# teamtomo/torch-motion-correction

Hardware: AMD Instinct MI355X
Metric: frames/sec motion-corrected, 40×4k×4k fp32 stack, 1/2/4/8 MI355X (higher is better)
Workload: dtype f32; 1 GPU; 40-frame 4096x4096 fp32 movie, global rigid shift estimate+correct (estimate_global_motion -> correct_motion, frames + sum out), 1 stack per GPU per step, consecutive steps overlapped on two HIP streams; b_factor=500

## Files before the change

### torch_motion_correction_amd/csrc/mc_wave_fft.h

```cpp
#pragma once

#ifdef __HIPCC__
#include "mc_common.h"
#define MC_HD __host__ __device__ __forceinline__
#else
#include <math.h>
#include <stdint.h>
struct cfloat {
  float x, y;
};
#define MC_HD static inline
#endif

typedef float wf2 __attribute__((ext_vector_type(2)));

#define WF_N 2048
#define WF_SLAB 1024

#ifdef __HIPCC__
__device__ __forceinline__ void wf_sync() {
  __builtin_amdgcn_fence(__ATOMIC_RELEASE, "wavefront");
  __builtin_amdgcn_wave_barrier();
  __builtin_amdgcn_fence(__ATOMIC_ACQUIRE, "wavefront");
}
// ... 49 lines not shown
  a2 = t0 - t2;
  a1 = wf_add_mi(t1, d);
  a3 = wf_sub_mi(t1, d);
}

MC_HD void wf_dft16(wf2 (&a)[16]) {
  const float C1 = 0.92387953251128673848f, S1 = 0.38268343236508978178f;
  const float H = 0.70710678118654752440f;
#pragma unroll
  for (int j = 0; j < 4; ++j) wf_bfly4(a[j], a[j + 4], a[j + 8], a[j + 12]);
  a[1 + 4] = wf_cmulc(a[1 + 4], C1, -S1);
  a[1 + 8] = wf_cmulc(a[1 + 8], H, -H);
  a[1 + 12] = wf_cmulc(a[1 + 12], S1, -C1);
  a[2 + 4] = wf_cmulc(a[2 + 4], H, -H);
  a[2 + 12] = wf_cmulc(a[2 + 12], -H, -H);
  a[3 + 4] = wf_cmulc(a[3 + 4], S1, -C1);
  a[3 + 8] = wf_cmulc(a[3 + 8], -H, -H);
  a[3 + 12] = wf_cmulc(a[3 + 12], -C1, S1);
#pragma unroll
  for (int p = 0; p < 4; ++p) {
    wf2 &b0 = a[4 * p], &b1 = a[4 * p + 1], &b2 = a[4 * p + 2], &b3 = a[4 * p + 3];
    if (p == 2) {
      const wf2 t0 = wf_add_mi(b0, b2), t1 = wf_sub_mi(b0, b2);
      const wf2 t2 = b1 + b3, d = b1 - b3;
      b0 = t0 + t2;
      b2 = t0 - t2;
      b1 = wf_add_mi(t1, d);
      b3 = wf_sub_mi(t1, d);
    } else {
      wf_bfly4(b0, b1, b2, b3);
    }
  }
#pragma unroll
  for (int p = 0; p < 4; ++p)
#pragma unroll
    for (int r = p + 1; r < 4; ++r) {
      const wf2 s = a[4 * p + r];
      a[4 * p + r] = a[4 * r + p];
      a[4 * r + p] = s;
    }
}

MC_HD void wf_dft16_lo2(wf2 (&a)[16]) {
  const float C1 = 0.92387953251128673848f, S1 = 0.38268343236508978178f;
  const float H = 0.70710678118654752440f;
  const wf2 x0 = a[0], x1 = a[1], x2 = a[14], x3 = a[15];
  a[0] = x0; a[4] = x0; a[8] = x0; a[12] = x0;
  a[1] = x1;
  a[1 + 4] = wf_cmulc(x1, C1, -S1);
  a[1 + 8] = wf_cmulc(x1, H, -H);
  a[1 + 12] = wf_cmulc(x1, S1, -C1);
  a[2] = x2;
  a[2 + 4] = wf_cmulc(x2, H, H);
  a[2 + 8] = -x2;
  a[2 + 12] = wf_cmulc(x2, -H, H);
  a[3] = x3;
  a[3 + 4] = wf_cmulc(x3, C1, S1);
  a[3 + 8] = wf_cmulc(x3, H, H);
  a[3 + 12] = wf_cmulc(x3, S1, C1);
#pragma unroll
  for (int p = 0; p < 4; ++p) {
    wf2 &b0 = a[4 * p], &b1 = a[4 * p + 1], &b2 = a[4 * p + 2], &b3 = a[4 * p + 3];
    if (p == 2) {
      const wf2 t0 = wf_add_mi(b0, b2), t1 = wf_sub_mi(b0, b2);
      const wf2 t2 = b1 + b3, d = b1 - b3;
      b0 = t0 + t2;
      b2 = t0 - t2;
      b1 = wf_add_mi(t1, d);
      b3 = wf_sub_mi(t1, d);
    } else {
      wf_bfly4(b0, b1, b2, b3);
    }
  }
#pragma unroll
  for (int p = 0; p < 4; ++p)
#pragma unroll
    for (int r = p + 1; r < 4; ++r) {
      const wf2 s = a[4 * p + r];
      a[4 * p + r] = a[4 * r + p];
      a[4 * r + p] = s;
    }
}

template <int KEEP>
MC_HD void wf_dft8_pruned(const wf2 (&e)[4], const wf2 (&o)[4], wf2 (&z)[8]) {
  const float H = 0.70710678118654752440f;
  wf2 e0 = e[0], e1 = e[1], e2 = e[2], e3 = e[3];
  wf2 o0 = o[0], o1 = o[1], o2 = o[2], o3 = o[3];
  wf_bfly4(e0, e1, e2, e3);
  wf_bfly4(o0, o1, o2, o3);
  z[0] = e0 + o0;
  z[7] = wf_fma_c(e3, o3, H, H);
  if (KEEP >= 2) {
    z[1] = wf_fma_c(e1, o1, H, -H);
    z[6] = wf_sub_mi(e2, o2);
  }
  if (KEEP >= 4) {
    z[2] = wf_add_mi(e2, o2);
    z[3] = wf_fma_c(e3, o3, -H, -H);
    z[4] = e0 - o0;
    z[5] = wf_fma_c(e1, o1, -H, H);
  }
}

struct WfLane {
  int x1w_base, x1w_mask;
  int x1r[4];
  int x2w;
  int x2r[4];
  int kbin[4];
  int self;
};

MC_HD WfLane wf_lane(int t) {
  WfLane L;
  {
    const int n2 = t >> 2, h1 = (t >> 1) & 1, h0 = t & 1;
    L.x1w_base = (n2 * 2 + h1) * 32 + h0 * 16;
    L.x1w_mask = (n2 & 3) | (h1 << 2) | (h0 << 3);
  }
  {
    const int k1 = t & 15, g2 = t >> 4, h1 = g2 >> 1, h0 = g2 & 1;
    const int lanepart = h1 * 32 + h0 * 16, lo = k1 ^ ((h1 << 2) | (h0 << 3));
    for (int v = 0; v < 4; ++v) L.x1r[v] = lanepart + (lo ^ v);
    L.x2w = g2 * 256 + k1;
  }
  L.kbin[0] = t;
  L.kbin[1] = t == 0 ? 128 : 256 - t;
  L.kbin[2] = 64 + t;
  L.kbin[3] = 192 - t;
  for (int s = 0; s < 4; ++s) L.x2r[s] = L.kbin[s];
  L.self = t == 0;
  return L;
}

MC_HD wf2 wf_unpack(wf2 zk, wf2 zmr, wf2 wk) {
  const wf2 zm = {zmr.x, -zmr.y};
  const wf2 sm = zk + zm, d = zk - zm;
  const wf2 wd = wf_cmul(d, wk);
  return wf_add_mi(sm, wd) * 0.5f;
}

template <int KEEP>
MC_HD void wf_unpack_lane(const wf2 (&z)[4][8], const wf2 (&wk)[4], bool self, wf2 (&X)[4][KEEP]) {
  const float C1 = 0.92387953251128673848f, S1 = 0.38268343236508978178f;
#pragma unroll
  for (int k3 = 0; k3 < KEEP; ++k3) {
    const wf2 m_a0 = self ? z[0][(8 - k3) & 7] : z[1][7 - k3];
    const wf2 m_a1 = self ? z[1][7 - k3] : z[0][7 - k3];
    wf2 w[4] = {wk[0], wk[1], wk[2], wk[3]};
    if (k3 == 1) {
#pragma unroll
      for (int s = 0; s < 4; ++s) w[s] = wf_cmulc(w[s], C1, -S1);
    }
    X[0][k3] = wf_unpack(z[0][k3], m_a0, w[0]);
    X[1][k3] = wf_unpack(z[1][k3], m_a1, w[1]);
    X[2][k3] = wf_unpack(z[2][k3], z[3][7 - k3], w[2]);
    X[3][k3] = wf_unpack(z[3][k3], z[2][7 - k3], w[3]);
  }
}

#define WF5_N 512
#define WF5_SLAB 512

MC_HD void wf_dft8(wf2 (&a)[8]) {
  const float H = 0.70710678118654752440f;
// ... 41 lines not shown
```

### torch_motion_correction_amd/csrc/xc_common.h

```cpp
#pragma once
#include <string.h>
#include "mc_fft.h"
#include "mcorr.h"

struct XcGeom {
  int W, H;
  int nkx;
  int kyp, kyn;
  int y0, ny;
  int x0, x1;
  int RG;
};

struct XcBox {
  int hl, hu, wl, wu;
};

__device__ __forceinline__ int kept_index(int ky, int H, int kyp, int kyn) {
  if (ky < kyp) return ky;
  if (ky >= H - kyn) return ky - (H - kyn) + kyp;
  return -1;
}

struct PeakCand {
  float v;
  int idx;
};
__device__ __forceinline__ void cand_merge(float& bv, int& bi, float v, int i) {
  if (v > bv || (v == bv && i < bi)) {
    bv = v;
    bi = i;
  }
}

__device__ __forceinline__ int float_order(float f) {
  const int i = __float_as_int(f);
  return i >= 0 ? i : i ^ 0x7fffffff;
}

#define MC_DISPATCH_CASE(V, ...) \
  case V: {                      \
    constexpr int L = V;         \
    __VA_ARGS__;                 \
  } break;
#define MC_DISPATCH_LOG(LOGV, ...)          \
  switch (LOGV) {                           \
    MC_DISPATCH_CASE(4, __VA_ARGS__)        \
    MC_DISPATCH_CASE(5, __VA_ARGS__)        \
    MC_DISPATCH_CASE(6, __VA_ARGS__)        \
    MC_DISPATCH_CASE(7, __VA_ARGS__)        \
    MC_DISPATCH_CASE(8, __VA_ARGS__)        \
    MC_DISPATCH_CASE(9, __VA_ARGS__)        \
    MC_DISPATCH_CASE(10, __VA_ARGS__)       \
    MC_DISPATCH_CASE(11, __VA_ARGS__)       \
    MC_DISPATCH_CASE(12, __VA_ARGS__)       \
    default:                                \
      return MC_ERR_UNSUPPORTED;            \
  }

static int geom_from(const mc_xc_geom* q, XcGeom* g, bool rows_pow2 = true, bool cols_pow2 = true) {
  if (!q) return MC_ERR_ARG;
  if (q->W < 4 || q->W > 16384 || ((q->W & 1) && q->W > 8191) || q->H < 2 || q->H > 8192) return MC_ERR_UNSUPPORTED;
  if (rows_pow2 && (!mc_is_pow2(q->W) || q->W < 32 || q->W > 8192)) return MC_ERR_UNSUPPORTED;
  if (cols_pow2 && (!mc_is_pow2(q->H) || q->H < 16 || q->H > 4096)) return MC_ERR_UNSUPPORTED;
  if (q->nkx < 1 || q->nkx > q->W / 2 + 1) return MC_ERR_ARG;
  if (q->kyp < 0 || q->kyn < 0 || q->kyp + q->kyn < 1 || q->kyp + q->kyn > q->H) return MC_ERR_ARG;
  if (q->RG < 1 || q->ny < 1 || q->ny % q->RG || q->H % q->RG) return MC_ERR_ARG;
  if (rows_pow2 && (q->RG % (MC_WG / fft_threads(q->W / 2)))) return MC_ERR_ARG;
  if (q->y0 < 0 || q->y0 + q->ny > q->H) return MC_ERR_ARG;
  if (q->x0 < 0 || q->x1 > q->W || q->x0 >= q->x1) return MC_ERR_ARG;
  if (!(q->W & 1) && ((q->x0 & 1) || (q->x1 & 1))) return MC_ERR_ARG;
  g->W = q->W; g->H = q->H; g->nkx = q->nkx; g->kyp = q->kyp; g->kyn = q->kyn;
  g->y0 = q->y0; g->ny = q->ny; g->x0 = q->x0; g->x1 = q->x1; g->RG = q->RG;
  return MC_OK;
}

static inline size_t rows_lds_bytes(int N, const XcGeom& g) {
  const int sgroups = MC_WG / fft_threads(N);
  return sizeof(cfloat) * ((size_t)sgroups * 2 * lds_len(N) + (size_t)g.nkx * (g.RG + 1));
}
template <typename Kernel>
static inline int mc_dyn_lds(Kernel kernel, size_t lds) {
  if (lds > 160 * 1024) return MC_ERR_ARG;
  if (lds > 64 * 1024)
    (void)hipFuncSetAttribute((const void*)kernel, hipFuncAttributeMaxDynamicSharedMemorySize, (int)lds);
  return MC_OK;
}

static inline int xc_near_groups(const XcGeom& g) {
  const int ngrp = g.H / g.RG, near = (64 + g.RG - 1) / g.RG;
  return 2 * near > ngrp ? ngrp / 2 : near;
}

void mc_launch_row_bounds(const cfloat* T2, float* bounds, int nkx, int H, int npairs, hipStream_t stream);
void mc_launch_peak_final(const float* part_val, const int* part_idx, int ngrp, int H, int W, int* peaks,
                          float* shifts, const int* shift_rows, int npairs, hipStream_t stream);

__attribute__((visibility("hidden"))) int mc_launch_cols_inv_near(const cfloat* S_cur, const int* cur_idx, const cfloat* S_ref, const int* ref_idx,
                            cfloat* T2n, float* bounds, const cfloat* tw_col, float scale, const XcGeom& g, int nstore,
                            int npairs, hipStream_t stream);
__attribute__((visibility("hidden"))) int mc_launch_cols_inv_gated(const cfloat* S_cur, const int* cur_idx, const cfloat* S_ref, const int* ref_idx,
                             cfloat* T2, const cfloat* tw_col, float scale, const XcGeom& g, const int* gate,
                             int npairs, hipStream_t stream);
```

### torch_motion_correction_amd/csrc/xc_rows_fwd.hip

```cpp
#include "xc_rows_fwd.h"

template <typename T>
__global__ __launch_bounds__(256) void xc_provisional_mean_kernel(const T* __restrict__ x, int n,
                                                                  float* __restrict__ m0) {
  double s = 0.0;
  for (int i = threadIdx.x; i < n; i += 256) s += (double)(float)x[i];
  for (int off = 32; off > 0; off >>= 1) s += __shfl_down(s, off);
  __shared__ double part[4];
  if ((threadIdx.x & 63) == 0) part[threadIdx.x >> 6] = s;
  __syncthreads();
  if (threadIdx.x == 0) {
    m0[0] = (float)(((part[0] + part[1]) + (part[2] + part[3])) / (double)n);
    m0[1] = 1.f;
    m0[2] = 1.f;
  }
}

__global__ void xc_stats_finalize(const double* __restrict__ acc_slots, double count,
                                  const float* __restrict__ m0, float* __restrict__ fix,
                                  float* __restrict__ out3) {
  double acc[2] = {0.0, 0.0};
  for (int s = 0; s < XC_STAT_SLOTS; ++s) {
    acc[0] += acc_slots[2 * s];
    acc[1] += acc_slots[2 * s + 1];
  }
  const double dm = acc[0] / count;
  double var = (acc[1] - acc[0] * acc[0] / count) / (count - 1.0);
  if (var < 0) var = 0;
  const float stdf = (float)sqrt(var);
  fix[0] = (float)dm;
  fix[1] = 1.0f / stdf;
  out3[0] = (float)((double)m0[0] + dm);
  out3[1] = 1.0f / stdf;
  out3[2] = stdf;
}

__global__ __launch_bounds__(256) void xc_rows_hot_fix(const long long* __restrict__ keys, const float2* __restrict__ rv,
                                                       int64_t n, int frame0, int njobs, int h, int w,
                                                       const float* __restrict__ mask,
                                                       const float* __restrict__ mean_rstd, cfloat* __restrict__ T1,
                                                       int W, int nkx, int y0, int ny) {
#pragma clang fp contract(off)
  const int64_t e0 = blockIdx.x;
  if (e0 >= n) return;
  const long long seg = keys[e0] / w;
  if (e0 > 0 && keys[e0 - 1] / w == seg) return;
  const int f = (int)(seg / h), y = (int)(seg - (long long)f * h);
  if (f < frame0 || f >= frame0 + njobs || y < y0 || y >= y0 + ny) return;
  const float rstd = mean_rstd[1];
  cfloat* col = T1 + (int64_t)(f - frame0) * nkx * ny + (y - y0);
  for (int kx = threadIdx.x; kx < nkx; kx += 256) {
    float ar = 0.f, ai = 0.f;
    for (int64_t e = e0; e < n && keys[e] / w == seg; ++e) {
      const int x = (int)(keys[e] - seg * w);
      const float m = mask ? mask[(int64_t)y * w + x] : 1.f;
      if (m == 0.f) continue;
      const float2 p = rv[e];
      const float dA = (p.x - p.y) * rstd * m;
      const int ph = (int)(((int64_t)kx * x) % W);
      const float rev = (float)ph / (float)W;
      ar += dA * __builtin_amdgcn_cosf(rev);
      ai -= dA * __builtin_amdgcn_sinf(rev);
    }
    cfloat* o = col + (int64_t)kx * ny;
    o->x += ar;
    o->y += ai;
  }
}

static int g_row_engine = 0;

enum K1Engine { K1_WAVE, K1_WG, K1_NONE };
static K1Engine k1_route(const XcGeom& g, int raw, bool half, const void* src, const float* gain, const float* mask,
                         const int* job_expo, int64_t row_stride, const XcBox& b, bool stats) {
  const bool shape = g.W == 2 * WF_N && g.nkx <= 512 && (g.ny % 8) == 0;
  const bool aligned16 = ((reinterpret_cast<uintptr_t>(src) | reinterpret_cast<uintptr_t>(gain) |
                           reinterpret_cast<uintptr_t>(mask)) & 15) == 0;
  if (raw) return shape && aligned16 && (row_stride & 7) == 0 ? K1_WAVE : K1_WG;
  const bool wave = shape && mask && !job_expo && aligned16 && (row_stride & 3) == 0 &&
                    (!stats || ((b.wl | b.wu) & 255) == 0);
  if (half && !wave) return K1_NONE;
  return wave && g_row_engine != 1 ? K1_WAVE : K1_WG;
}

static K1WaveVariant k1_wave_variant(const XcGeom& g, int raw, bool half, const int* row_chord) {
  const bool inner = g.x0 >= 256 && g.x0 <= 512 && g.x1 >= 3584 && g.x1 <= 3840;
  if (half) return K1WaveVariant{g.nkx <= 256, K1_LOADS_HALF};
  if (raw || !inner) return K1WaveVariant{g.nkx <= 256, K1_LOADS_ALL};
  return K1WaveVariant{g.nkx <= 256, row_chord ? K1_LOADS_INNER_CHORD : K1_LOADS_INNER};
}

static bool wave512_shape(const XcGeom& g, const float* mask) {
  return g.W == 2 * WF5_N && g.nkx <= 128 && (g.ny % 8) == 0 && (reinterpret_cast<uintptr_t>(mask) & 7) == 0;
}

extern "C" {

int mc_xc_row_engine(int mode) {
  if (mode < 0 || mode > 1) return MC_ERR_ARG;
  g_row_engine = mode;
  return MC_OK;
}

int mc_xc_rows_lds_bytes(const mc_xc_geom* q) {
  XcGeom g;
  int rc = geom_from(q, &g, true, false);
  if (rc) return rc;
  return (int)rows_lds_bytes(g.W / 2, g);
}

static int rows_forward_impl(const float* src, const int64_t* job_off, int64_t row_stride,
                             const int* job_expo, const float* mask, const float* mean_rstd,
                             void* T1, const void* tw_row, int njobs, const mc_xc_geom* q,
                             const XcBox* box, double* stats_acc, void* stream,
                             const int* row_chord = nullptr, bool half = false) {
  XcGeom g;
  int rc = geom_from(q, &g, true, false);
  if (rc) return rc;
  if (!src || !job_off || !T1 || !tw_row || njobs < 1) return MC_ERR_ARG;
  const XcBox b = box ? *box : XcBox{0, 0, 0, 0};
  switch (k1_route(g, 0, half, src, nullptr, mask, job_expo, row_stride, b, stats_acc != nullptr)) {
    case K1_NONE: return MC_ERR_UNSUPPORTED;
    case K1_WG:
      return k1_wg_launch(0, src, job_off, row_stride, job_expo, mask, mean_rstd, T1, tw_row, njobs, g, b, stats_acc,
                          nullptr, nullptr, stream);
    default:
      return k1_wave_launch(k1_wave_variant(g, 0, half, row_chord), 0, src, job_off, row_stride, mask, mean_rstd, T1,
                            tw_row, njobs, g, b, stats_acc, row_chord, nullptr, nullptr, stream);
  }
}

int mc_xc_rows_forward_dual_t(const void* src, int storage, const int64_t* job_off, int64_t row_stride,
                              const int* expo_a, const int* expo_b, const float* mask,
                              const float* mean_rstd, void* T1a, void* T1b, const void* tw_row,
                              int njobs, const mc_xc_geom* q, const int* row_chord, void* stream) {
  if (storage != MC_STORE_F32 && storage != MC_STORE_F16) return MC_ERR_UNSUPPORTED;
  XcGeom g;
  int rc = geom_from(q, &g, true, false);
  if (rc) return rc;
  if (!src || !job_off || !expo_a || !mask || !T1a || !tw_row || njobs < 1 || (expo_b && !T1b))
    return MC_ERR_ARG;
  if (!wave512_shape(g, mask)) return MC_ERR_UNSUPPORTED;
  return k1_wave512_launch(storage, src, job_off, row_stride, expo_a, expo_b, mask, mean_rstd, T1a, T1b, tw_row, njobs,
                           g, row_chord, nullptr, 1, nullptr, stream);
}

int mc_xc_rows_forward_dual_raw(const void* raw, int storage, const float* gain, int64_t frame_area,
                                const int64_t* job_off, int64_t row_stride, const int* expo_a, const int* expo_b,
                                const float* mask, const float* job_sub, const float* mean_rstd, void* T1a, void* T1b,
                                const void* tw_row, int njobs, const mc_xc_geom* q, const int* row_chord,
                                void* stream) {
  if (storage != MC_STORE_U8 && storage != MC_STORE_I16) return MC_ERR_UNSUPPORTED;
  XcGeom g;
  int rc = geom_from(q, &g, true, false);
  if (rc) return rc;
  if (!raw || !gain || !job_off || !expo_a || !mask || !job_sub || !mean_rstd || !T1a || !tw_row || njobs < 1 ||
      (expo_b && !T1b) || frame_area < 1 || row_stride < 1)
    return MC_ERR_ARG;
  if (!wave512_shape(g, mask) || (reinterpret_cast<uintptr_t>(gain) & 3) ||
      (storage == MC_STORE_I16 && (reinterpret_cast<uintptr_t>(raw) & 1)))
    return MC_ERR_UNSUPPORTED;
  return k1_wave512_launch(storage, raw, job_off, row_stride, expo_a, expo_b, mask, mean_rstd, T1a, T1b, tw_row, njobs,
                           g, row_chord, gain, frame_area, job_sub, stream);
}

int mc_xc_rows_forward(const float* src, const int64_t* job_off, int64_t row_stride,
                       const int* job_expo, const float* mask, const float* mean_rstd,
// ... 72 lines not shown
```

### torch_motion_correction_amd/csrc/xc_rows_fwd_wave.hip

```cpp
#include "xc_rows_fwd.h"


__device__ __forceinline__ void wf_pin(int& v, float dep) { asm volatile("" : "+v"(v) : "v"(dep)); }

#define WF_TWA (4 * 128)
#define WF_TWB (4 * 15 * 2)
constexpr int WF_ROWS_PER_WG = 32;
constexpr int WF_MIN_WG = 2;

template <int N1LO, int N1HI, bool CLAMP_ALL, bool HALF = false, int RAW = 0>
__device__ __forceinline__ void wf_load_px(const void* __restrict__ row_any, int t, int xlo, int xhi,
                                           float4 (&px)[16]) {
  if constexpr (RAW == 1) {
    const unsigned char* row = static_cast<const unsigned char*>(row_any);
#pragma unroll
    for (int n1 = N1LO; n1 < N1HI; ++n1) {
      const int x = 256 * n1 + 4 * t;
      const int xs = (CLAMP_ALL || n1 == N1LO || n1 == N1HI - 1) ? min(max(x, xlo), xhi) : x;
      px[n1].x = __builtin_nontemporal_load(reinterpret_cast<const float*>(row + xs));
    }
    return;
  }
  if constexpr (HALF || RAW == 2) {
    const _Float16* row = static_cast<const _Float16*>(row_any);
#pragma unroll
    for (int n1 = N1LO; n1 < N1HI; ++n1) {
      const int x = 256 * n1 + 4 * t;
      typedef float f2 __attribute__((ext_vector_type(2)));
      const int xs = (CLAMP_ALL || n1 == N1LO || n1 == N1HI - 1) ? min(max(x, xlo), xhi) : x;
      const f2 q = __builtin_nontemporal_load(reinterpret_cast<const f2*>(row + xs));
      px[n1].x = q.x;
      px[n1].y = q.y;
    }
    return;
  }
  const float* row = static_cast<const float*>(row_any);
#pragma unroll
  for (int n1 = N1LO; n1 < N1HI; ++n1) {
    const int x = 256 * n1 + 4 * t;
    typedef float f4 __attribute__((ext_vector_type(4)));
    const int xs = (CLAMP_ALL || n1 == N1LO || n1 == N1HI - 1) ? min(max(x, xlo), xhi) : x;
    const f4 q = __builtin_nontemporal_load(reinterpret_cast<const f4*>(row + xs));
    px[n1] = make_float4(q.x, q.y, q.z, q.w);
  }
}

template <int N1LO, int N1HI>
__device__ __forceinline__ void wf_load_mask(const float* __restrict__ mrow, int t, float4 (&mk)[16]) {
#pragma unroll
  for (int n1 = N1LO; n1 < N1HI; ++n1) mk[n1] = *reinterpret_cast<const float4*>(mrow + 256 * n1 + 4 * t);
}

__device__ __forceinline__ wf2 wf_unpack_h2(float bits) {
  const unsigned v = __float_as_uint(bits);
  return wf2{(float)__builtin_bit_cast(_Float16, (unsigned short)(v & 0xffffu)),
             (float)__builtin_bit_cast(_Float16, (unsigned short)(v >> 16))};
}

__device__ __forceinline__ void wf_unpack_u8x4(float bits, wf2& a01, wf2& a23) {
  const unsigned v = __float_as_uint(bits);
  a01 = wf2{(float)(v & 0xffu), (float)((v >> 8) & 0xffu)};
  a23 = wf2{(float)((v >> 16) & 0xffu), (float)(v >> 24)};
}
__device__ __forceinline__ wf2 wf_unpack_i16x2(float bits) {
  const unsigned v = __float_as_uint(bits);
  return wf2{(float)(short)(v & 0xffffu), (float)((int)v >> 16)};
}

template <int KEEP, bool STATS, int N1LO, int N1HI, bool CLAMP_ALL, bool HALF = false, int RAW = 0>
__device__ __forceinline__ void wf_row(float4 (&px)[16], float4 (&mk)[16], const float* __restrict__ mrow,
                                       const void* __restrict__ next_row, int t, wf2* slab,
                                       const cfloat* twA, const cfloat* twB, const cfloat* twK,
                                       const XcGeom& g, int box_lo, int box_hi, float mean, float rstd,
                                       float& st_s, float& st_q, wf2 (&X)[4][KEEP], int xlo, int xhi,
                                       int nxlo, int nxhi, const float* __restrict__ grow = nullptr) {
  wf2 A0[16], A1[16];
  if constexpr (RAW != 0) {
    auto half_row = [&](auto lo_tag) {
      constexpr int LO = decltype(lo_tag)::value, HI = LO + 8;
      float4 gq[8], mq[8];
#pragma unroll
      for (int n1 = LO; n1 < HI; ++n1) {
        if (n1 >= N1LO && n1 < N1HI) {
          const int x = 256 * n1 + 4 * t;
          const int xs = (CLAMP_ALL || n1 == N1LO || n1 == N1HI - 1) ? min(max(x, xlo), xhi) : x;
          gq[n1 - LO] = *reinterpret_cast<const float4*>(grow + xs);
          mq[n1 - LO] = *reinterpret_cast<const float4*>(mrow + x);
        }
      }
// ... 316 lines not shown
```

### torch_motion_correction_amd/csrc/xc_search.hip

```cpp
#include "xc_common.h"

__global__ void xc_search_init(int* __restrict__ best, int* __restrict__ gate, float* __restrict__ bounds,
                               int npairs, int nbounds, float* __restrict__ shift_table, int nshift) {
  const int i = blockIdx.x * blockDim.x + threadIdx.x;
  if (i < nbounds) bounds[i] = 0.f;
  if (i < nshift) shift_table[i] = 0.f;
  if (i < npairs) best[i] = (int)0x807fffffu;
  if (i == 0) gate[0] = 0;
}

__global__ void xc_far_needed(const float* __restrict__ bounds, const int* __restrict__ best,
                              float* __restrict__ part_val, int* __restrict__ part_idx,
                              int* __restrict__ need_full, int H, int RG, int near) {
  const int ngrp = H / RG;
  const int p = blockIdx.y;
  const int grp = near + blockIdx.x * blockDim.x + threadIdx.x;
  if (grp >= ngrp - near) return;
  float b = 0.f;
  for (int r = 0; r < RG; ++r) b = fmaxf(b, bounds[(int64_t)p * H + grp * RG + r]);
  b = b * 1.0001f + 1e-30f;
  part_val[(int64_t)p * ngrp + grp] = -INFINITY;
  part_idx[(int64_t)p * ngrp + grp] = 0x7fffffff;
  const int fb = __float_as_int(b);
  if ((fb >= 0 ? fb : fb ^ 0x7fffffff) >= best[p]) atomicOr(need_full, 1);
}



__global__ __launch_bounds__(256) void xc_row_bounds(const cfloat* __restrict__ T2,
                                                     float* __restrict__ bounds, int nkx, int H) {
  __shared__ float part[4][64];
  const int ly = threadIdx.x & 63, slice = threadIdx.x >> 6;
  const int y = blockIdx.x * 64 + ly;
  const int p = blockIdx.y;
  float b0 = 0.f, b1 = 0.f, b2 = 0.f, b3 = 0.f;
  if (y < H) {
    const cfloat* in = T2 + (int64_t)p * nkx * H + y;
    int kx = slice;
    for (; kx + 12 < nkx; kx += 16) {
      const cfloat v0 = in[(int64_t)kx * H], v1 = in[(int64_t)(kx + 4) * H];
      const cfloat v2 = in[(int64_t)(kx + 8) * H], v3 = in[(int64_t)(kx + 12) * H];
      b0 += (kx == 0 ? 1.f : 2.f) * sqrtf(v0.x * v0.x + v0.y * v0.y);
      b1 += 2.f * sqrtf(v1.x * v1.x + v1.y * v1.y);
      b2 += 2.f * sqrtf(v2.x * v2.x + v2.y * v2.y);
      b3 += 2.f * sqrtf(v3.x * v3.x + v3.y * v3.y);
    }
    for (; kx < nkx; kx += 4) {
      const cfloat v = in[(int64_t)kx * H];
      b0 += (kx == 0 ? 1.f : 2.f) * sqrtf(v.x * v.x + v.y * v.y);
    }
  }
  part[slice][ly] = (b0 + b1) + (b2 + b3);
  __syncthreads();
  if (slice == 0 && y < H)
    bounds[(int64_t)p * H + y] = (part[0][ly] + part[1][ly]) + (part[2][ly] + part[3][ly]);
}

template <int LOGN, int EPI>
__global__ __launch_bounds__(MC_WG) void xc_rows_inv(const cfloat* __restrict__ T2,
                                                     const float* __restrict__ bounds,
                                                     int* __restrict__ best,
                                                     float* __restrict__ part_val,
                                                     int* __restrict__ part_idx,
                                                     float* __restrict__ out_real,
                                                     const int64_t* __restrict__ out_off,
                                                     int64_t out_stride,
                                                     const cfloat* __restrict__ tw_row, XcGeom g,
                                                     int near, int phase, int compact,
                                                     const int* __restrict__ gate) {
  constexpr int N = 1 << LOGN;
  if (gate && gate[0] == 0) return;
  constexpr int NT = fft_threads(N), SG = MC_WG / NT;
  constexpr int R0 = FftPlan<N>::radix(0), NB0 = N / R0, IT0 = (NB0 + NT - 1) / NT;
  extern __shared__ __attribute__((aligned(16))) char smem[];
  const int tid = threadIdx.x;
  const int lt = tid & (NT - 1), sg = tid / NT;
  cfloat* l0 = reinterpret_cast<cfloat*>(smem) + sg * 2 * lds_len(N);
  cfloat* l1 = l0 + lds_len(N);
  cfloat* stg = reinterpret_cast<cfloat*>(smem) + SG * 2 * lds_len(N);
  const int p = blockIdx.y;
  const int RG = g.RG;
  const int ngrp = g.H / RG;
  int grp = blockIdx.x;
// ... 24 lines not shown
    for (int u = 0; u < 8; ++u) {
      const int i = i0 + u * MC_WG;
      const int kx = i / RG, r = i - kx * RG;
      if (i < g.nkx * RG) v8[u] = in[(int64_t)kx * cstride + r];
    }
#pragma unroll
    for (int u = 0; u < 8; ++u) {
      const int i = i0 + u * MC_WG;
      const int kx = i / RG, r = i - kx * RG;
      if (i < g.nkx * RG) stg[kx * (RG + 1) + r] = v8[u];
    }
  }
  FftTwiddles<N> T;
  T.template init<+1>(lt, tw_row, 2);
  cfloat wk[IT0][R0];
#pragma unroll
  for (int it = 0; it < IT0; ++it)
#pragma unroll
    for (int q = 0; q < R0; ++q) {
      const int j = lt + it * NT;
      const int k = (NB0 % NT == 0 || j < NB0) ? j + q * NB0 : 0;
      cfloat w = tw_row[k];
      w.y = -w.y;
      wk[it][q] = w;
    }
  __syncthreads();
  float bv = -INFINITY;
  int bi = 0x7fffffff;
  int s = 0;
  for (int r = sg; r < RG; r += SG) {
    const int y = grp * RG + r;
    auto load = [&](int k, int it, int q) {
      const int km = N - k;
      cfloat xk = (k < g.nkx) ? stg[k * (RG + 1) + r] : cmake(0.f, 0.f);
      cfloat xm = (km < g.nkx) ? cconj(stg[km * (RG + 1) + r]) : cmake(0.f, 0.f);
      if (k == 0) {
        xk.y = 0.f;
        xm.y = 0.f;
      }
      const cfloat sm = cadd(xk, xm), d = csub(xk, xm);
      const cfloat wd = cmul(wk[it][q], d);
      return cmake(sm.x - wd.y, sm.y + wd.x);
    };
    int res;
    if constexpr (EPI == 0) {
      auto store = [&](int n, cfloat v) {
        const int flat = y * g.W + 2 * n;
        cand_merge(bv, bi, v.x, flat);
        cand_merge(bv, bi, v.y, flat + 1);
      };
      res = wg_fft_pp<N, +1, true>(l0, l1, s, lt, T, load, store);
    } else {
      float* orow = out_real + out_off[p] + (int64_t)y * out_stride;
      auto store = [&](int n, cfloat v) {
        orow[2 * n] = v.x;
        orow[2 * n + 1] = v.y;
      };
      res = wg_fft_pp<N, +1, true>(l0, l1, s, lt, T, load, store);
    }
    s = res ^ 1;
  }
  if constexpr (EPI == 0) {
    for (int off = 32; off > 0; off >>= 1) {
      const float ov = __shfl_down(bv, off);
      const int oi = __shfl_down(bi, off);
      cand_merge(bv, bi, ov, oi);
    }
    __shared__ float wv[MC_WG / 64];
    __shared__ int wi[MC_WG / 64];
    if ((tid & 63) == 0) {
      wv[tid >> 6] = bv;
      wi[tid >> 6] = bi;
    }
    __syncthreads();
    if (tid == 0) {
      for (int w = 1; w < MC_WG / 64; ++w) cand_merge(bv, bi, wv[w], wi[w]);
      part_val[(int64_t)p * ngrp + grp] = bv;
      part_idx[(int64_t)p * ngrp + grp] = bi;
      atomicMax(&best[p], float_order(bv));
    }
  }
}

__global__ void xc_peak_final(const float* __restrict__ part_val, const int* __restrict__ part_idx,
                              int ngrp, int H, int W, int* __restrict__ peaks,
                              float* __restrict__ shifts, const int* __restrict__ shift_rows) {
  const int p = blockIdx.x;
  float bv = -INFINITY;
  int bi = 0x7fffffff;
  for (int i = threadIdx.x; i < ngrp; i += blockDim.x)
    cand_merge(bv, bi, part_val[(int64_t)p * ngrp + i], part_idx[(int64_t)p * ngrp + i]);
  for (int off = 32; off > 0; off >>= 1) {
    const float ov = __shfl_down(bv, off);
    const int oi = __shfl_down(bi, off);
    cand_merge(bv, bi, ov, oi);
  }
  if (threadIdx.x == 0) {
    if (bi == 0x7fffffff) bi = 0;
    peaks[p] = bi;
    const int py = bi / W, px = bi - py * W;
    const int row = shift_rows ? shift_rows[p] : p;
    shifts[2 * row] = (float)(py <= H / 2 ? py : py - H);
    shifts[2 * row + 1] = (float)(px <= W / 2 ? px : px - W);
  }
}

template <int LOGN>
__global__ __launch_bounds__(MC_WG) void xc_peak_nbhd(const cfloat* __restrict__ T2,
                                                      const int* __restrict__ peaks,
                                                      float* __restrict__ nb,
                                                      const cfloat* __restrict__ tw_row, XcGeom g,
                                                      const cfloat* __restrict__ T2n,
                                                      const int* __restrict__ gate, int nstore) {
  constexpr int N = 1 << LOGN;
  __shared__ __attribute__((aligned(16))) cfloat line[lds_len(N)];
  const int tid = threadIdx.x;
  const int p = blockIdx.y, dy = (int)blockIdx.x - 1;
  const int pk = peaks[p];
  const int py = pk / g.W, px = pk - py * g.W;
  const int y = py + dy;
  float* o = nb + (int64_t)p * 9 + (dy + 1) * 3;
  if (y < 0 || y >= g.H) {
    if (tid < 3) o[tid] = __builtin_nanf("");
    return;
  }
  const cfloat* in = T2 + (int64_t)p * g.nkx * g.H + y;
  int64_t cs = g.H;
  if (T2n && gate[0] == 0) {
    const int yn = y < nstore ? y : y - (g.H - 2 * nstore);
    if (yn < 0 || yn >= 2 * nstore || (y >= nstore && y < g.H - nstore)) {
      if (tid < 3) o[tid] = __builtin_nanf("");
      return;
    }
    cs = 2 * nstore;
    in = T2n + (int64_t)p * g.nkx * cs + yn;
  }
  auto X = [&](int k) { return in[(int64_t)k * cs]; };
  auto load = [&](int k) {
    const int km = N - k;
    cfloat xk = (k < g.nkx) ? X(k) : cmake(0.f, 0.f);
    cfloat xm = (km < g.nkx) ? cconj(X(km)) : cmake(0.f, 0.f);
    if (k == 0) {
      xk.y = 0.f;
      xm.y = 0.f;
    }
    const cfloat s = cadd(xk, xm), d = csub(xk, xm);
    cfloat w = tw_row[k];
    w.y = -w.y;
    const cfloat wd = cmul(w, d);
    return cmake(s.x - wd.y, s.y + wd.x);
  };
  auto store = [&](int n, cfloat v) { line[lpad(n)] = v; };
  wg_fft<N, +1>(line, tid, tw_row, 2, load, store);
  __syncthreads();
  if (tid < 3) {
    const int x = px + tid - 1;
    float v = __builtin_nanf("");
    if (x >= 0 && x < g.W) {
      const cfloat z = line[lpad(x >> 1)];
      v = (x & 1) ? z.y : z.x;
    }
    o[tid] = v;
  }
}

void mc_launch_row_bounds(const cfloat* T2, float* bounds, int nkx, int H, int npairs, hipStream_t stream) {
// ... 16 lines not shown
}
static void rows_argmax_launch(RowsInvKernel k, size_t lds, int ngroups, int npairs, const void* T2, const float* bounds,
                               int* best, float* part_val, int* part_idx, const void* tw_row, const XcGeom& g,
                               int near, int phase, int compact, const int* gate, hipStream_t stream) {
  hipLaunchKernelGGL(k, dim3(ngroups, npairs), dim3(MC_WG), lds, stream, (const cfloat*)T2, bounds, best, part_val,
                     part_idx, (float*)nullptr, (const int64_t*)nullptr, (int64_t)0, (const cfloat*)tw_row, g, near,
                     phase, compact, gate);
}

extern "C" {

int mc_xc_rows_inverse_argmax(const void* T2, float* part_val, int* part_idx, int* peaks,
                              float* shifts, const void* tw_row, int npairs, const mc_xc_geom* q,
                              void* stream) {
  XcGeom g;
  int rc = geom_from(q, &g, true, false);
  if (rc) return rc;
  if (!T2 || !part_val || !part_idx || !peaks || !shifts || !tw_row || npairs < 1)
    return MC_ERR_ARG;
  hipStream_t st = (hipStream_t)stream;
  RowsInvKernel k;
  size_t lds;
  if ((rc = rows_inv_kernel<0>(g, &k, &lds))) return rc;
  const int ngrp = g.H / g.RG;
  int* best = part_idx + (int64_t)npairs * ngrp;
  {
    const float ninf = -INFINITY;
    int pat;
    memcpy(&pat, &ninf, 4);
    pat = pat >= 0 ? pat : pat ^ 0x7fffffff;
    hipError_t e = hipMemsetD32Async((hipDeviceptr_t)best, pat, npairs, st);
    if (e != hipSuccess) return (int)e;
  }
  const int near = xc_near_groups(g), nfar = ngrp - 2 * near;
  float* bounds = part_val + (int64_t)npairs * ngrp;
  if (nfar > 0) mc_launch_row_bounds((const cfloat*)T2, bounds, g.nkx, g.H, npairs, st);
  if (near > 0)
    rows_argmax_launch(k, lds, 2 * near, npairs, T2, bounds, best, part_val, part_idx, tw_row, g, near, 0, 0, nullptr, st);
  if (nfar > 0)
    rows_argmax_launch(k, lds, nfar, npairs, T2, bounds, best, part_val, part_idx, tw_row, g, near, 1, 0, nullptr, st);
  rc = mc_check_launch();
  if (rc) return rc;
  mc_launch_peak_final(part_val, part_idx, ngrp, g.H, g.W, peaks, shifts, nullptr, npairs, st);
  return mc_check_launch();
}

int mc_xc_near_rows(const mc_xc_geom* q) {
  XcGeom g;
  int rc = geom_from(q, &g, true, true);
  if (rc) return rc;
  return xc_near_groups(g) * g.RG + XC_NEAR_GUARD;
}

int mc_xc_correlate_argmax(const void* S_cur, const int* cur_idx, const void* S_ref,
                           const int* ref_idx, void* T2_full, void* T2_near, float* part_val,
                           int* part_idx, int* peaks, float* shifts, const int* shift_rows,
                           int n_shift_rows, float* nb, const void* tw_col, const void* tw_row,
                           float scale, int npairs, const mc_xc_geom* q, void* stream) {
  XcGeom g;
  int rc = geom_from(q, &g, true, true);
  if (rc) return rc;
  if (!S_cur || !cur_idx || !S_ref || !ref_idx || !T2_full || !T2_near || !part_val || !part_idx ||
      !peaks || !shifts || !tw_col || !tw_row || npairs < 1)
    return MC_ERR_ARG;
  if (g.H < 1024) return MC_ERR_UNSUPPORTED;
  hipStream_t st = (hipStream_t)stream;
  RowsInvKernel k;
  size_t lds;
  if ((rc = rows_inv_kernel<0>(g, &k, &lds))) return rc;
  const int ngrp = g.H / g.RG;
  const int near = xc_near_groups(g);
  if (near < 1) return MC_ERR_UNSUPPORTED;
  const int nstore = near * g.RG + XC_NEAR_GUARD;
  if (nstore > 256) return MC_ERR_UNSUPPORTED;
  int* best = part_idx + (int64_t)npairs * ngrp;
  int* gate = best + npairs;
  float* bounds = part_val + (int64_t)npairs * ngrp;
  if (shift_rows && n_shift_rows < 1) return MC_ERR_ARG;
  hipLaunchKernelGGL(xc_search_init, dim3((npairs * g.H + 255) / 256), dim3(256), 0, st, best, gate, bounds,
                     npairs, npairs * g.H, shifts, shift_rows ? 2 * n_shift_rows : 0);
  rc = mc_launch_cols_inv_near((const cfloat*)S_cur, cur_idx, (const cfloat*)S_ref, ref_idx, (cfloat*)T2_near, bounds,
                               (const cfloat*)tw_col, scale, g, nstore, npairs, st);
  if (rc) return rc;
  rows_argmax_launch(k, lds, 2 * near, npairs, T2_near, bounds, best, part_val, part_idx, tw_row, g, near, 0,
                     1 + XC_NEAR_GUARD, nullptr, st);
  rc = mc_check_launch();
  if (rc) return rc;
  const int nfar = ngrp - 2 * near;
  if (nfar > 0) {
    hipLaunchKernelGGL(xc_far_needed, dim3((nfar + 63) / 64, npairs), dim3(64), 0, st,
                       (const float*)bounds, (const int*)best, part_val, part_idx, gate, g.H, g.RG, near);
    rc = mc_launch_cols_inv_gated((const cfloat*)S_cur, cur_idx, (const cfloat*)S_ref, ref_idx, (cfloat*)T2_full,
                                  (const cfloat*)tw_col, scale, g, gate, npairs, st);
    if (rc) return rc;
    rows_argmax_launch(k, lds, nfar, npairs, T2_full, bounds, best, part_val, part_idx, tw_row, g, near, 1, 0, gate, st);
    rc = mc_check_launch();
    if (rc) return rc;
  }
  mc_launch_peak_final(part_val, part_idx, ngrp, g.H, g.W, peaks, shifts, shift_rows, npairs, st);
  if (nb) {
    MC_DISPATCH_LOG(mc_ilog2(g.W) - 1, {
      hipLaunchKernelGGL(xc_peak_nbhd<L>, dim3(3, npairs), dim3(MC_WG), 0, st, (const cfloat*)T2_full,
                         (const int*)peaks, nb, (const cfloat*)tw_row, g, (const cfloat*)T2_near,
                         (const int*)gate, nstore);
    });
  }
  return mc_check_launch();
}

int mc_xc_rows_inverse_store(const void* T2, float* out, const int64_t* out_off,
                             int64_t out_stride, const void* tw_row, int nframes,
                             const mc_xc_geom* q, void* stream) {
  XcGeom g;
  int rc = geom_from(q, &g, true, false);
  if (rc) return rc;
  if (!T2 || !out || !out_off || !tw_row || nframes < 1) return MC_ERR_ARG;
  RowsInvKernel k;
  size_t lds;
  if ((rc = rows_inv_kernel<1>(g, &k, &lds))) return rc;
  hipLaunchKernelGGL(k, dim3(g.H / g.RG, nframes), dim3(MC_WG), lds, (hipStream_t)stream, (const cfloat*)T2,
                     (const float*)nullptr, (int*)nullptr, (float*)nullptr, (int*)nullptr, out, out_off, out_stride,
                     (const cfloat*)tw_row, g, 0, 0, 0, (const int*)nullptr);
  return mc_check_launch();
}

int mc_xc_peak_neighbourhood(const void* T2, const int* peaks, float* nb, const void* tw_row,
                             int npairs, const mc_xc_geom* q, void* stream) {
  XcGeom g;
  int rc = geom_from(q, &g, true, false);
  if (rc) return rc;
  if (!T2 || !peaks || !nb || !tw_row || npairs < 1) return MC_ERR_ARG;
  const int logn = mc_ilog2(g.W) - 1;
  dim3 grid(3, npairs);
  MC_DISPATCH_LOG(logn, {
    hipLaunchKernelGGL(xc_peak_nbhd<L>, grid, dim3(MC_WG), 0, (hipStream_t)stream,
                       (const cfloat*)T2, peaks, nb, (const cfloat*)tw_row, g, (const cfloat*)nullptr,
                       (const int*)nullptr, 0);
  });
  return mc_check_launch();
}

}
```

Before: 25000 frames/s.

## Add wavefront-level pruned inverse row FFT argmax kernel for near cross-correlation groups

Measured after the change: 25200 frames/s, median of 6. About the same (+0.8%).

```diff
diff --git a/torch_motion_correction_amd/csrc/mc_wave_fft.h b/torch_motion_correction_amd/csrc/mc_wave_fft.h
--- a/torch_motion_correction_amd/csrc/mc_wave_fft.h
+++ b/torch_motion_correction_amd/csrc/mc_wave_fft.h
@@ -155,6 +155,81 @@
     }
 }
 
+MC_HD void wf_dft16_lo4(wf2 (&a)[16]) {
+  const float C1 = 0.92387953251128673848f, S1 = 0.38268343236508978178f;
+  const float H = 0.70710678118654752440f;
+#pragma unroll
+  for (int j = 0; j < 4; ++j) {
+    const wf2 x0 = a[j], x3 = a[j + 12];
+    a[j] = x0 + x3;
+    a[j + 4] = wf_sub_mi(x0, x3);
+    a[j + 8] = x0 - x3;
+    a[j + 12] = wf_add_mi(x0, x3);
+  }
+  a[1 + 4] = wf_cmulc(a[1 + 4], C1, -S1);
+  a[1 + 8] = wf_cmulc(a[1 + 8], H, -H);
+  a[1 + 12] = wf_cmulc(a[1 + 12], S1, -C1);
+  a[2 + 4] = wf_cmulc(a[2 + 4], H, -H);
+  a[2 + 12] = wf_cmulc(a[2 + 12], -H, -H);
+  a[3 + 4] = wf_cmulc(a[3 + 4], S1, -C1);
+  a[3 + 8] = wf_cmulc(a[3 + 8], -H, -H);
+  a[3 + 12] = wf_cmulc(a[3 + 12], -C1, S1);
+#pragma unroll
+  for (int p = 0; p < 4; ++p) {
+    wf2 &b0 = a[4 * p], &b1 = a[4 * p + 1], &b2 = a[4 * p + 2], &b3 = a[4 * p + 3];
+    if (p == 2) {
+      const wf2 t0 = wf_add_mi(b0, b2), t1 = wf_sub_mi(b0, b2);
+      const wf2 t2 = b1 + b3, d = b1 - b3;
+      b0 = t0 + t2;
+      b2 = t0 - t2;
+      b1 = wf_add_mi(t1, d);
+      b3 = wf_sub_mi(t1, d);
+    } else {
+      wf_bfly4(b0, b1, b2, b3);
+    }
+  }
+#pragma unroll
+  for (int p = 0; p < 4; ++p)
+#pragma unroll
+    for (int r = p + 1; r < 4; ++r) {
+      const wf2 s = a[4 * p + r];
+      a[4 * p + r] = a[4 * r + p];
+      a[4 * r + p] = s;
+    }
+}
+
+template <int KI>
+MC_HD int wf_inv_n1(int j) { return j < KI ? j : 16 - 2 * KI + j; }
+MC_HD int wf_inv_src(int n) { return n < WF_N / 2 ? n : WF_N - n; }
+MC_HD wf2 wf_inv_pack(wf2 x, wf2 wcq, int n1) {
+  const float C[16] = {1.f, 0.98078528040323044913f, 0.92387953251128675613f, 0.83146961230254523708f,
+                       0.70710678118654752440f, 0.55557023301960222474f, 0.38268343236508977173f,
+                       0.19509032201612826785f, 0.f, -0.19509032201612826785f, -0.38268343236508977173f,
+                       -0.55557023301960222474f, -0.70710678118654752440f, -0.83146961230254523708f,
+                       -0.92387953251128675613f, -0.98078528040323044913f};
+  const float S[16] = {0.f, 0.19509032201612826785f, 0.38268343236508977173f, 0.55557023301960222474f,
+                       0.70710678118654752440f, 0.83146961230254523708f, 0.92387953251128675613f,
+                       0.98078528040323044913f, 1.f, 0.98078528040323044913f, 0.92387953251128675613f,
+                       0.83146961230254523708f, 0.70710678118654752440f, 0.55557023301960222474f,
+                       0.38268343236508977173f, 0.19509032201612826785f};
+  const wf2 wc = n1 == 0 ? wcq : wf_cmulc(wcq, C[n1], S[n1]);
+  if (n1 < 8) {
+    const wf2 wd = wf_cmul(x, wc);
+    return wf2{x.x - wd.y, -x.y - wd.x};
+  }
+  const wf2 xm = {x.x, -x.y};
+  const wf2 wd = wf_cmul(xm, wc);
+  return wf2{xm.x + wd.y, wd.x - xm.y};
+}
+
+#define WF_TWA (4 * 128)
+#define WF_TWB (4 * 15 * 2)
+MC_HD int wf_table_src(int i) {
+  if (i < WF_TWA) return (2 * (i & 127)) << (i >> 7);
+  const int e = i - WF_TWA, h = e & 1, k2 = ((e >> 1) % 15) + 1, gq = e / 30;
+  return 32 * (2 * gq + h) * k2;
+}
+
 template <int KEEP>
 MC_HD void wf_dft8_pruned(const wf2 (&e)[4], const wf2 (&o)[4], wf2 (&z)[8]) {
   const float H = 0.70710678118654752440f;
diff --git a/torch_motion_correction_amd/csrc/xc_common.h b/torch_motion_correction_amd/csrc/xc_common.h
--- a/torch_motion_correction_amd/csrc/xc_common.h
+++ b/torch_motion_correction_amd/csrc/xc_common.h
@@ -96,6 +96,8 @@
 void mc_launch_peak_final(const float* part_val, const int* part_idx, int ngrp, int H, int W, int* peaks,
                           float* shifts, const int* shift_rows, int npairs, hipStream_t stream);
 
+__attribute__((visibility("hidden"))) bool k4_wave_route(const XcGeom& g, const void* T2n, int nstore, int guard);
+
 __attribute__((visibility("hidden"))) int mc_launch_cols_inv_near(const cfloat* S_cur, const int* cur_idx, const cfloat* S_ref, const int* ref_idx,
                             cfloat* T2n, float* bounds, const cfloat* tw_col, float scale, const XcGeom& g, int nstore,
                             int npairs, hipStream_t stream);
diff --git a/torch_motion_correction_amd/csrc/xc_rows_fwd.hip b/torch_motion_correction_amd/csrc/xc_rows_fwd.hip
--- a/torch_motion_correction_amd/csrc/xc_rows_fwd.hip
+++ b/torch_motion_correction_amd/csrc/xc_rows_fwd.hip
@@ -83,6 +83,11 @@
   return wave && g_row_engine != 1 ? K1_WAVE : K1_WG;
 }
 
+bool k4_wave_route(const XcGeom& g, const void* T2n, int nstore, int guard) {
+  const bool shape = g.W == 2 * WF_N && g.nkx <= 512 && (g.RG % 8) == 0 && ((nstore + guard) & 1) == 0;
+  return shape && (reinterpret_cast<uintptr_t>(T2n) & 15) == 0 && g_row_engine != 1;
+}
+
 static K1WaveVariant k1_wave_variant(const XcGeom& g, int raw, bool half, const int* row_chord) {
   const bool inner = g.x0 >= 256 && g.x0 <= 512 && g.x1 >= 3584 && g.x1 <= 3840;
   if (half) return K1WaveVariant{g.nkx <= 256, K1_LOADS_HALF};
diff --git a/torch_motion_correction_amd/csrc/xc_rows_fwd_wave.hip b/torch_motion_correction_amd/csrc/xc_rows_fwd_wave.hip
--- a/torch_motion_correction_amd/csrc/xc_rows_fwd_wave.hip
+++ b/torch_motion_correction_amd/csrc/xc_rows_fwd_wave.hip
@@ -3,8 +3,6 @@
 
 __device__ __forceinline__ void wf_pin(int& v, float dep) { asm volatile("" : "+v"(v) : "v"(dep)); }
 
-#define WF_TWA (4 * 128)
-#define WF_TWB (4 * 15 * 2)
 constexpr int WF_ROWS_PER_WG = 32;
 constexpr int WF_MIN_WG = 2;
 
diff --git a/torch_motion_correction_amd/csrc/xc_search.hip b/torch_motion_correction_amd/csrc/xc_search.hip
--- a/torch_motion_correction_amd/csrc/xc_search.hip
+++ b/torch_motion_correction_amd/csrc/xc_search.hip
@@ -1,4 +1,5 @@
 #include "xc_common.h"
+#include "mc_wave_fft.h"
 
 __global__ void xc_search_init(int* __restrict__ best, int* __restrict__ gate, float* __restrict__ bounds,
                                int npairs, int nbounds, float* __restrict__ shift_table, int nshift) {
@@ -189,6 +190,183 @@
   }
 }
 
+constexpr int K4_WAVE_MIN_WG = 2;
+template <int KI>
+__device__ __forceinline__ void k4_wave_load(const cfloat* __restrict__ in, int cstride, int nkx, int t, int pair,
+                                             float4 (&P)[4 * KI]) {
+#pragma unroll
+  for (int j = 0; j < 2 * KI; ++j)
+#pragma unroll
+    for (int h = 0; h < 2; ++h) {
+      const int kx = wf_inv_src(128 * wf_inv_n1<KI>(j) + 2 * t + h);
+      P[2 * j + h] = *reinterpret_cast<const float4*>(in + (int64_t)min(kx, nkx - 1) * cstride + 2 * pair);
+    }
+}
+
+template <int KI>
+__global__ __launch_bounds__(256, K4_WAVE_MIN_WG) void xc_rows_inv_wave(const cfloat* __restrict__ T2n, int* __restrict__ best,
+                                                        float* __restrict__ part_val, int* __restrict__ part_idx,
+                                                        const cfloat* __restrict__ tw_row, XcGeom g, int near,
+                                                        int guard) {
+  __shared__ __attribute__((aligned(16))) cfloat slabs[4][WF_SLAB];
+  __shared__ __attribute__((aligned(16))) cfloat tab[WF_TWA + WF_TWB];
+  __shared__ float wv_val[4];
+  __shared__ int wv_idx[4];
+  const cfloat* twA = tab;
+  const cfloat* twB = tab + WF_TWA;
+  const int t = threadIdx.x & 63;
+  const int wv = __builtin_amdgcn_readfirstlane(threadIdx.x >> 6);
+  wf2* slab = reinterpret_cast<wf2*>(slabs[wv]);
+  {
+    constexpr int NTAB = WF_TWA + WF_TWB, PER = (NTAB + 255) / 256;
+    cfloat tv[PER];
+#pragma unroll
+    for (int j = 0; j < PER; ++j) {
+      const int i = threadIdx.x + 256 * j;
+      tv[j] = tw_row[wf_table_src(i < NTAB ? i : NTAB - 1)];
+    }
+#pragma unroll
+    for (int j = 0; j < PER; ++j) {
+      const int i = threadIdx.x + 256 * j;
+      if (i < NTAB) tab[i] = tv[j];
+    }
+  }
+  const int p = blockIdx.y, RG = g.RG, ngrp = g.H / RG, bx = blockIdx.x;
+  const int grp = bx < near ? bx : ngrp - 2 * near + bx;
+  const int nstore = near * RG + guard, cstride = 2 * nstore;
+  const int coff = bx < near ? bx * RG : nstore + guard + (bx - near) * RG;
+  const cfloat* in = T2n + (int64_t)p * g.nkx * cstride + coff;
+  cfloat c0 = tw_row[2 * t], c1 = tw_row[2 * t + 1];
+  const wf2 wcq0 = {c0.x, -c0.y}, wcq1 = {c1.x, -c1.y};
+  const int npairs_wave = RG / 8;
+  float4 P[4 * KI];
+  k4_wave_load<KI>(in, cstride, g.nkx, t, wv, P);
+  __syncthreads();
+  float bv = -INFINITY;
+  int bi = 0x7fffffff;
+#pragma unroll 1
+  for (int i = 0; i < 2 * npairs_wave; ++i) {
+    const int pair = wv + 4 * (i >> 1), second = i & 1;
+    const int y = grp * RG + 2 * pair + second;
+    wf2 A0[16], A1[16];
+#pragma unroll
+    for (int n1 = 0; n1 < 16; ++n1) {
+      A0[n1] = wf2{0.f, 0.f};
+      A1[n1] = wf2{0.f, 0.f};
+    }
+#pragma unroll
+    for (int j = 0; j < 2 * KI; ++j) {
+      const int n1 = wf_inv_n1<KI>(j);
+      const int k0 = wf_inv_src(128 * n1 + 2 * t), k1 = wf_inv_src(128 * n1 + 2 * t + 1);
+      const float4 q0 = P[2 * j], q1 = P[2 * j + 1];
+      wf2 x0 = second ? wf2{q0.z, q0.w} : wf2{q0.x, q0.y};
+      wf2 x1 = second ? wf2{q1.z, q1.w} : wf2{q1.x, q1.y};
+      if (n1 == 0 && t == 0) x0.y = 0.f;
+      if (k0 >= g.nkx) x0 = wf2{0.f, 0.f};
+      if (k1 >= g.nkx) x1 = wf2{0.f, 0.f};
+      A0[n1] = wf_inv_pack(x0, wcq0, n1);
+      A1[n1] = wf_inv_pack(x1, wcq1, n1);
+    }
+    if (second && i + 1 < 2 * npairs_wave) {
+      int tp = t;
+      asm volatile("" : "+v"(tp) : "v"(A1[15].y));
+      k4_wave_load<KI>(in, cstride, g.nkx, tp, pair + 4, P);
+    }
+    int tl = t;
+    asm volatile("" : "+v"(tl) : "v"(A0[15].x));
+    const WfLane L = wf_lane(tl);
+    if constexpr (KI == 2) wf_dft16_lo2(A0); else wf_dft16_lo4(A0);
+    {
+      const float4* twa = reinterpret_cast<const float4*>(twA) + tl;
+      float4 w[4];
+#pragma unroll
+      for (int sb = 0; sb < 4; ++sb) w[sb] = twa[sb * 64];
+      if constexpr (KI == 2) wf_dft16_lo2(A1); else wf_dft16_lo4(A1);
+      wf_twiddle16(A0, wf2{w[0].x, w[0].y}, wf2{w[1].x, w[1].y}, wf2{w[2].x, w[2].y}, wf2{w[3].x, w[3].y});
+      wf_twiddle16(A1, wf2{w[0].z, w[0].w}, wf2{w[1].z, w[1].w}, wf2{w[2].z, w[2].w}, wf2{w[3].z, w[3].w});
+    }
+    wf2 B0[16], B1[16];
+#pragma unroll
+    for (int k1 = 0; k1 < 16; ++k1) slab[L.x1w_base + (k1 ^ L.x1w_mask)] = A0[k1];
+    wf_sync();
+#pragma unroll
+    for (int n2 = 0; n2 < 16; ++n2) B0[n2] = slab[L.x1r[n2 & 3] + 64 * n2];
+    wf_sync();
+#pragma unroll
+    for (int k1 = 0; k1 < 16; ++k1) slab[L.x1w_base + (k1 ^ L.x1w_mask)] = A1[k1];
+    wf_sync();
+    wf_dft16(B0);
+#pragma unroll
+    for (int n2 = 0; n2 < 16; ++n2) B1[n2] = slab[L.x1r[n2 & 3] + 64 * n2];
+    wf_sync();
+    {
+      const float4* twb = reinterpret_cast<const float4*>(twB) + (tl >> 4) * 15;
+      float4 w[15];
+#pragma unroll
+      for (int k2 = 1; k2 < 16; ++k2) w[k2 - 1] = twb[k2 - 1];
+      wf_dft16(B1);
+#pragma unroll
+      for (int k2 = 1; k2 < 16; ++k2) {
+        B0[k2] = wf_cmul(B0[k2], wf2{w[k2 - 1].x, w[k2 - 1].y});
+        B1[k2] = wf_cmul(B1[k2], wf2{w[k2 - 1].z, w[k2 - 1].w});
+      }
+    }
+#pragma unroll
+    for (int k2 = 0; k2 < 16; ++k2) slab[L.x2w + 16 * k2] = B0[k2];
+    wf_sync();
+    wf2 Ce[4][4], Co[4][4];
+#pragma unroll
+    for (int s = 0; s < 4; ++s)
+#pragma unroll
+      for (int n3h = 0; n3h < 4; ++n3h) Ce[s][n3h] = slab[L.x2r[s] + 256 * n3h];
+    wf_sync();
+#pragma unroll
+    for (int k2 = 0; k2 < 16; ++k2) slab[L.x2w + 16 * k2] = B1[k2];
+    wf_sync();
+#pragma unroll
+    for (int s = 0; s < 4; ++s)
+#pragma unroll
+      for (int n3h = 0; n3h < 4; ++n3h) Co[s][n3h] = slab[L.x2r[s] + 256 * n3h];
+    wf_sync();
+    wf2 z[4][8];
+    float m = -INFINITY;
+#pragma unroll
+    for (int s = 0; s < 4; ++s) {
+      wf_dft8_pruned<4>(Ce[s], Co[s], z[s]);
+#pragma unroll
+      for (int k3 = 0; k3 < 8; ++k3) {
+        z[s][k3].y = -z[s][k3].y;
+        m = fmaxf(m, fmaxf(z[s][k3].x, z[s][k3].y));
+      }
+    }
+    for (int off = 32; off > 0; off >>= 1) m = fmaxf(m, __shfl_xor(m, off));
+    if (m >= bv) {
+      int ri = 0x7fffffff;
+#pragma unroll
+      for (int s = 0; s < 4; ++s)
+#pragma unroll
+        for (int k3 = 0; k3 < 8; ++k3) {
+          const int flat = y * g.W + 2 * (L.kbin[s] + 256 * k3);
+          if (z[s][k3].x == m) ri = min(ri, flat);
+          if (z[s][k3].y == m) ri = min(ri, flat + 1);
+        }
+      for (int off = 32; off > 0; off >>= 1) ri = min(ri, __shfl_xor(ri, off));
+      if (ri != 0x7fffffff) cand_merge(bv, bi, m, ri);
+    }
+  }
+  if (t == 0) {
+    wv_val[wv] = bv;
+    wv_idx[wv] = bi;
+  }
+  __syncthreads();
+  if (threadIdx.x == 0) {
+    for (int w = 1; w < 4; ++w) cand_merge(bv, bi, wv_val[w], wv_idx[w]);
+    part_val[(int64_t)p * ngrp + grp] = bv;
+    part_idx[(int64_t)p * ngrp + grp] = bi;
+    atomicMax(&best[p], float_order(bv));
+  }
+}
+
 __global__ void xc_peak_final(const float* __restrict__ part_val, const int* __restrict__ part_idx,
                               int ngrp, int H, int W, int* __restrict__ peaks,
                               float* __restrict__ shifts, const int* __restrict__ shift_rows) {
@@ -371,8 +549,14 @@
   rc = mc_launch_cols_inv_near((const cfloat*)S_cur, cur_idx, (const cfloat*)S_ref, ref_idx, (cfloat*)T2_near, bounds,
                                (const cfloat*)tw_col, scale, g, nstore, npairs, st);
   if (rc) return rc;
-  rows_argmax_launch(k, lds, 2 * near, npairs, T2_near, bounds, best, part_val, part_idx, tw_row, g, near, 0,
-                     1 + XC_NEAR_GUARD, nullptr, st);
+  if (k4_wave_route(g, T2_near, nstore, XC_NEAR_GUARD)) {
+    auto kw = g.nkx <= 256 ? xc_rows_inv_wave<2> : xc_rows_inv_wave<4>;
+    hipLaunchKernelGGL(kw, dim3(2 * near, npairs), dim3(256), 0, st, (const cfloat*)T2_near, best, part_val, part_idx,
+                       (const cfloat*)tw_row, g, near, XC_NEAR_GUARD);
+  } else {
+    rows_argmax_launch(k, lds, 2 * near, npairs, T2_near, bounds, best, part_val, part_idx, tw_row, g, near, 0,
+                       1 + XC_NEAR_GUARD, nullptr, st);
+  }
   rc = mc_check_launch();
   if (rc) return rc;
   const int nfar = ngrp - 2 * near;
```
